# ten2net/Gym-Trading-Env

Measured on AMD Instinct MI355X. Metric: env-steps/sec, higher is better.
Workload: dtype f64

## Files before the change

gym-trading-env_amd/batched.py:

```python
from __future__ import annotations

import ctypes as C

import numpy as np

from . import _abi, spaces, staging
from .batched_history import history_column, history_columns
from .config import make_config

_NP = {"int32": np.int32, "float64": np.float64}


def _as_staged(ds, n_dyn, name="Stock"):
    if isinstance(ds, staging.StagedDataset):
        return ds
    if isinstance(ds, tuple) and len(ds) in (2, 4):
        return staging.stage_arrays(ds[0], ds[1], n_dyn=n_dyn, name=name,
                                    high=ds[2] if len(ds) == 4 else None,
                                    low=ds[3] if len(ds) == 4 else None)
    return staging.stage_dataframe(ds, n_dyn=n_dyn, name=name)


def _device_view(ptr, shape, typestr, device, strides=None):
    import torch
# ... 1102 lines not shown
                raise ValueError(f"expected rule_of_env of shape ({self.num_envs},)")
        torch.cuda.current_stream(dev).synchronize()
        _abi.check(self._lib, self._lib.gte_bind_exit_rules(
            self._h, C.c_void_p(d_rules.data_ptr()), R, None if d_map is None else C.c_void_p(d_map.data_ptr()),
            C.byref(ptr)))
        self._exits = (d_rules, d_map)
        self._exit_state_ptr = int(ptr.value or 0)

    @property
    def num_exit_rules(self) -> int:
        return int(self._exits[0].shape[0]) if self._exits else 0

    def exit_state(self):
        from .exit_state import ExitState
        if not self._exit_state_ptr:
            raise ValueError("exit_state() before bind_exits(): the env has no exit state yet")
        return ExitState(self, self._exit_state_ptr)

    def synchronize(self):
        _abi.check(self._lib, self._lib.gte_synchronize(self._h))

    def launch_info(self) -> dict:
        v = [C.c_int32() for _ in range(4)]
        _abi.check(self._lib, self._lib.gte_get_launch_info(self._h, *[C.byref(x) for x in v]))
        d = dict(zip(("envs_per_wave", "threads_per_block", "n_blocks", "vector_bytes"),
                     (x.value for x in v)))
        flags, d["vector_bytes"] = divmod(d["vector_bytes"], 1000)
        d["phase_a"] = "cooperative" if flags & 1 else "per-wave"
        d["dyn_columns"] = ("global", "lds-raw-rings", "lds-resolved")[(flags >> 1) & 3]
        d["structure"] = "phase A, LDS barrier, gather"
        d["obs_stores"] = ("plain", "non-temporal", "sc1", "?")[(flags >> 4) & 3]
        d["resident_workgroups_per_cu"] = (flags >> 6) & 15
        d["slide_obs_stores"] = ("plain", "non-temporal", "sc1", "?")[(flags >> 10) & 3]
        return d

    def timer_start(self):
        _abi.check(self._lib, self._lib.gte_timer_start(self._h))

    def timer_mark(self):
        _abi.check(self._lib, self._lib.gte_timer_stop(self._h, None))

    def timer_stop(self) -> float:
        ms = C.c_float()
        _abi.check(self._lib, self._lib.gte_timer_stop(self._h, C.byref(ms)))
        return ms.value

    def close(self, **kwargs):
        if getattr(self, "_h", None) and self._h.value:
            self._lib.gte_destroy(self._h)
            self._h = C.c_void_p()
        self.closed = True

    def __del__(self):
        try:
            self.close()
        except Exception:
            pass
```

gym-trading-env_amd/csrc/gte_api.hip:

```cpp
#include <hip/hip_runtime.h>

#include <climits>
#include <cstdarg>
#include <cstdio>
#include <cstdlib>
#include <cstring>
#include <new>
#include <string>
#include <utility>
#include <vector>

#include "gte_launch.h"
#include "gte_ledger.h"

using gte::DatasetDesc;
using gte::EnvRec;
using gte::Params;
using gte_ledger::FLAGS;
using gte_ledger::WINDOW;
using gte_ledger::ledger;

static thread_local std::string g_err = "";

static int fail(int code, const char* fmt, ...) {
  char buf[512];
  va_list ap;
  va_start(ap, fmt);
  vsnprintf(buf, sizeof buf, fmt, ap);
  va_end(ap);
  g_err = buf;
  return code;
}

#define HIPCHK(expr)                                                              \
  do {                                                                            \
    hipError_t e_ = (expr);                                                       \
    if (e_ != hipSuccess)                                                         \
      return fail(e_ == hipErrorOutOfMemory ? GTE_ERR_OOM : GTE_ERR_HIP,          \
                  "%s failed: %s", #expr, hipGetErrorString(e_));                 \
  } while (0)

enum { SLIDE_AB_ORDER = 1, SLIDE_AB_STORE = 2 };

struct LaunchPlan {
  int vec = 1, blocks = 0, threads = 256;
  bool coop = false;
  int stage = 0;
  int hot_per_cu = 0;
  int store = 0;
  int slide_store = 0;
  bool hot_tu = false;
  bool fused_log = false;
  bool always_dense = false;
  int slide_rows = 0;
  bool full_windows = false;
  int slide_ab = 0;
  bool fused_rollout = false;
  bool resident_rollout = false;
  int affinity_period = 0;
  int n_bins_per_ds = 0;
  int state_epw = 0;
  int rollout_epw = 0;
  int resident_slots[3] = {0, 0, 0};
  int resident_epb[3] = {0, 0, 0};
};

struct gte_env {
  gte_config cfg;
  Params p;
  hipStream_t stream = nullptr;
  hipStream_t own_stream = nullptr;
  hipEvent_t ev0 = nullptr, ev1 = nullptr;
  std::vector<void*> allocs;
  std::vector<DatasetDesc> h_ds;
  std::vector<void*> ds_allocs[4];
  DatasetDesc* d_ds = nullptr;
  gte_outputs owned;
  int32_t* d_actions = nullptr;
  uint8_t* d_mask = nullptr;
  int32_t *d_inj_idx = nullptr, *d_inj_pos = nullptr, *d_inj_ds = nullptr;
  int32_t *d_q_idx = nullptr, *d_q_pos = nullptr, *d_q_ds = nullptr;
  double* d_lo_limit_in = nullptr;
  uint8_t* d_lo_persist_in = nullptr;
// ... 241 lines not shown
  int nb = 8192 / p.D;
  if (const char* o = getenv("GTE_AFFINITY_BINS")) nb = atoi(o) / p.D;
  nb = nb < 1 ? 1 : (nb > 4096 ? 4096 : nb);
  L.n_bins_per_ds = nb;
  TRY(dev_alloc(E, &E->d_perm, N, false));
  TRY(dev_alloc(E, &E->d_slot_of_rank, N, false));
  TRY(dev_alloc(E, &E->d_bins, (size_t)2 * p.D * nb));
  if (hipMemcpy(E->d_slot_of_rank, slot_of_rank.data(), sizeof(int32_t) * N, hipMemcpyHostToDevice) !=
      hipSuccess)
    return fail(GTE_ERR_HIP, "copying slot_of_rank failed");
  L.affinity_period = period;
  return GTE_OK;
}

static int slide_store_policy(const gte_env* E) {
  const LaunchPlan& L = E->plan;
  const Params& p = E->p;
  if (L.slide_rows == 0 || L.full_windows || (L.slide_ab & SLIDE_AB_STORE)) return L.store;
  int s = E->cfg.nontemporal_obs;
  if (s == 3) s = ((size_t)p.N * (p.W + L.slide_rows) * p.Fobs * sizeof(float) > ((size_t)190 << 20)) ? 1 : L.store;
  if (s != L.store && L.hot_tu && s != 0) {
    hipDeviceProp_t prop;
    const size_t smem = gte::lds_bytes(p, L.stage);
    const int per_cu = s == 1 ? gte::hot_blocks_per_cu_nt(smem) : gte::hot_blocks_per_cu(smem);
    if (hipGetDeviceProperties(&prop, E->cfg.device) != hipSuccess || prop.multiProcessorCount <= 0 ||
        per_cu < (L.blocks + prop.multiProcessorCount - 1) / prop.multiProcessorCount)
      s = L.store;
  }
  if (const char* o = getenv("GTE_SLIDE_STORE"))
    if (o[0] >= '0' && o[0] <= '2' && o[1] == '\0') s = o[0] - '0';
  return s;
}

static int plan_launches(gte_env* E) {
  LaunchPlan& L = E->plan;
  Params& p = E->p;
  const gte_config& cfg = E->cfg;
  const int kv = cfg.kernel_variant;
  L.store = cfg.nontemporal_obs;
  if (L.store == 3) L.store = ((size_t)p.N * p.W * p.Fobs * sizeof(float) > ((size_t)190 << 20)) ? 1 : 2;
  step_geometry(E, !(kv & (GTE_KV_PER_WAVE_PHASE_A | GTE_KV_NO_LDS_STAGING)), !(kv & GTE_KV_GENERIC_COPY));
  p.debug = cfg.debug_flags;
  L.coop = (p.epw * GTE_WAVES <= 64) && !(kv & GTE_KV_PER_WAVE_PHASE_A);
  L.stage = (p.nd > 0 && gte::lds_bytes(p, 1) <= 48 * 1024 && !(kv & GTE_KV_NO_LDS_STAGING)) ? (p.persist ? 2 : 1) : 0;
  p.lean_rows = (L.vec == 4 && L.stage == 1 && !(kv & GTE_KV_GENERIC_COPY)) ? 1 : 0;
  p.hot_lds = (kv & GTE_KV_RECORD_DIRECT) ? 0 : 1;
  const bool hot_shape = L.vec == 4 && L.coop && L.stage == 1;
  L.hot_tu = hot_shape && !(kv & GTE_KV_SHARED_TU);
  L.fused_log = cfg.log_steps > 0 && !(kv & GTE_KV_LOG_SEPARATE);
  L.always_dense = (kv & GTE_KV_DENSE_FLAGS) != 0;
  L.slide_rows = 0;
  if (hot_shape && (int64_t)p.W * p.Fobs / 4 >= 64 && p.has_window && !p.persist && !cfg.final_obs &&
      cfg.log_steps == 0 && cfg.obs_slack_rows >= 0)
    L.slide_rows = cfg.obs_slack_rows > 0 ? cfg.obs_slack_rows : 2 * p.W / 5;
  L.full_windows = getenv("GTE_SLIDE_FULL_WINDOWS") != nullptr;
  if (const char* o = getenv("GTE_SLIDE_AB")) L.slide_ab = atoi(o);
  L.slide_store = slide_store_policy(E);
  L.fused_rollout = hot_shape && !cfg.final_obs && cfg.log_steps == 0 && !(kv & GTE_KV_ROLLOUT_PER_STEP);
  L.resident_rollout = p.W >= 2 && !(kv & GTE_KV_ROLLOUT_GATHER);
  L.state_epw = (p.N >= 64 * 1024) ? 64 : 32;
  return setup_affinity(E);
}

extern "C" {

int gte_abi_version(void) { return GTE_ABI_VERSION; }

const char* gte_last_error(void) { return g_err.c_str(); }

int gte_device_count(void) {
  int n = 0;
  if (hipGetDeviceCount(&n) != hipSuccess) return 0;
  return n;
}

int gte_create(const gte_config* cfg, gte_env** out) {
  if (!out) return fail(GTE_ERR_INVALID, "out is NULL");
  *out = nullptr;
  TRY(validate(cfg));
  TRY(require_device(cfg->device));
  HIPCHK(hipSetDevice(cfg->device));
  gte_env* E = new (std::nothrow) gte_env();
  if (!E) return fail(GTE_ERR_OOM, "host allocation failed");
  E->cfg = *cfg;
  memset(&E->p, 0, sizeof(Params));
  memset(&E->owned, 0, sizeof(gte_outputs));
  Params& p = E->p;
  p.N = cfg->n_envs;
  p.D = cfg->n_datasets;
  p.Fs = cfg->n_static;
// ... 351 lines not shown
  const bool slide = slides_own && !capturing && ledger().holds(E, WINDOW, {obs}) && E->p.obs_head < L.slide_rows;
  const bool env_order = slide && !L.full_windows && !(L.slide_ab & SLIDE_AB_ORDER);
  if (env_order) { if (L.affinity_period > 0) E->steps_since_rebuild += 1; }
  else TRY(age_order(E, 1));
  Params p = E->p;
  if (env_order) p.perm = nullptr;
  if (terminal_rec) p.final_rec = terminal_rec;
  p.actions = t.actions; p.obs = t.obs; p.reward = t.reward; p.reward64 = t.reward64;
  p.terminated = t.terminated; p.truncated = t.truncated;
  if (!t.own_obs) {
    p.obs_rows = p.W; p.obs_head = 0;
    obs = {t.obs, sizeof(float) * (size_t)p.N * p.W * p.Fobs};
  } else if (E->sliding) {
    if (slide) {
      E->p.obs_head += 1;
      if (p.persist || p.final_obs)
        return fail(GTE_ERR_STATE, "internal: a sliding step with dyn_persist or final_obs (plan_launches grants neither)");
      p.slide = L.full_windows ? 0 : 1;
    } else {
      E->p.obs_head = 0;
    }
    p.obs_head = E->p.obs_head;
  }
  advance_term_slot(E, p);
  if (L.fused_log) {
    p.log = E->log;
    p.log_cursor = E->log_cursor + (E->term_slot ^ 1);
  }
  const gte_ledger::Span term = flag_span(E, p.terminated), trunc = flag_span(E, p.truncated);
  p.flags_sparse = !capturing && !L.always_dense && ledger().holds(E, FLAGS, {term, trunc}) ? 1 : 0;
  ledger().wrote(E, {obs, term, trunc}, capturing, FLAGS | WINDOW);
  const bool hot = L.hot_tu && gte::hot_tu_covers(p);
  if (p.slide) store = L.slide_store;
  if (hot && store == 2)
    HIPCHK(gte::launch_step_hot(p, L.blocks, L.threads, gte::lds_bytes(p, L.stage), E->stream));
  else if (hot && store == 1)
    HIPCHK(gte::launch_step_hot_nt(p, L.blocks, L.threads, gte::lds_bytes(p, L.stage), E->stream));
  else
    HIPCHK(gte::launch_step(p, L.vec, store, L.coop, L.stage, L.blocks, L.threads, E->stream));
  ledger().establish(E, FLAGS, {term, trunc}, capturing);
  if (slides_own) ledger().establish(E, WINDOW, {obs}, capturing);
  if (L.fused_log) E->log_rows += 1;
  else TRY(append_log(E, p));
  return GTE_OK;
}

int gte_step(gte_env* E, const int32_t* actions, int32_t actions_on_device) {
  if (!E) return fail(GTE_ERR_INVALID, "env is NULL");
  if (!E->was_reset) return fail(GTE_ERR_STATE, "gte_step before gte_reset");
  if (!actions) return fail(GTE_ERR_INVALID, "actions is NULL");
  const bool capturing = stream_capturing(E);
  if (capturing && !actions_on_device)
    return fail(GTE_ERR_STATE, "gte_step on a capturing stream needs device-resident actions "
                               "(a copy from pageable host memory cannot be captured)");
  if (!actions_on_device) {
    TRY(stage(E, E->d_actions, actions, sizeof(int32_t) * (size_t)E->p.N));
    actions = E->d_actions;
  }
  return enqueue_step(E, own_targets(E, actions), E->plan.store, capturing);
}

int gte_get_schedule(gte_env* E, gte_schedule* out) {
  if (!E || !out) return fail(GTE_ERR_INVALID, "NULL argument");
  out->log_rows = E->log_rows;
  out->term_slot = E->term_slot;
  out->steps_since_rebuild = E->steps_since_rebuild;
  return GTE_OK;
// ... 997 lines not shown
  if (!E || !host_dst) return fail(GTE_ERR_INVALID, "NULL argument");
  const Params& p = E->p;
  if (first_env < 0 || n < 0 || (int64_t)first_env + n > p.N)
    return fail(GTE_ERR_INVALID, "env range [%d, %d) out of [0, %d)", first_env, first_env + n, p.N);
  const size_t per = (size_t)p.W * p.Fobs;
  if (!p.obs) return fail(GTE_ERR_STATE, "gte_read_obs before gte_reset (no observation exists yet)");
  HIPCHK(hipStreamSynchronize(E->stream));
  const size_t stride = (size_t)obs_env_stride(p);
  const float* src = obs_window0(p) + stride * first_env;
  if (stride == per || n == 0)
    HIPCHK(hipMemcpy(host_dst, src, sizeof(float) * per * n, hipMemcpyDeviceToHost));
  else
    HIPCHK(hipMemcpy2D(host_dst, sizeof(float) * per, src, sizeof(float) * stride, sizeof(float) * per, (size_t)n,
                       hipMemcpyDeviceToHost));
  return GTE_OK;
}

int gte_copy_to_host(gte_env* E, const void* device_src, void* host_dst, uint64_t bytes) {
  if (!E || !device_src || !host_dst) return fail(GTE_ERR_INVALID, "NULL argument");
  HIPCHK(hipStreamSynchronize(E->stream));
  HIPCHK(hipMemcpy(host_dst, device_src, (size_t)bytes, hipMemcpyDeviceToHost));
  return GTE_OK;
}

int gte_get_launch_info(gte_env* E, int32_t* envs_per_wave, int32_t* threads_per_block,
                        int32_t* n_blocks, int32_t* vector_bytes) {
  if (!E) return fail(GTE_ERR_INVALID, "env is NULL");
  if (envs_per_wave) *envs_per_wave = E->p.epw;
  const LaunchPlan& L = E->plan;
  if (threads_per_block) *threads_per_block = L.threads;
  if (n_blocks) *n_blocks = L.blocks;
  if (vector_bytes)
    *vector_bytes = L.vec * 4 + 1000 * ((L.coop ? 1 : 0) + 2 * L.stage + 16 * L.store + 64 * (L.hot_per_cu & 15) +
                                        1024 * (E->sliding ? L.slide_store : L.store));
  return GTE_OK;
}

#ifdef GTE_STAMPS
int gte_debug_set_stamps(gte_env* E, void* device_buf) {
  if (!E) return fail(GTE_ERR_INVALID, "env is NULL");
  E->p.inj_ds = (const int32_t*)device_buf;
  return GTE_OK;
}
#endif

void gte_destroy(gte_env* E) {
  if (!E) return;
  (void)hipSetDevice(E->cfg.device);
  (void)gte_comm_destroy(E);
  (void)hipStreamSynchronize(E->stream);
  if (E->own_stream) (void)hipStreamSynchronize(E->own_stream);
  for (void* ptr : E->allocs) if (ptr) (void)hipFree(ptr);
  for (auto& v : E->ds_allocs)
    for (void* ptr : v)
      if (ptr) (void)hipFree(ptr);
  for (int32_t* q : {E->d_q_idx, E->d_q_pos, E->d_q_ds})
    if (q) (void)hipFree(q);
  if (E->h_snap) (void)hipHostFree(E->h_snap);
  if (E->h_logpack) (void)hipHostFree(E->h_logpack);
  if (E->ev0) (void)hipEventDestroy(E->ev0);
  if (E->ev1) (void)hipEventDestroy(E->ev1);
  if (E->own_stream) (void)hipStreamDestroy(E->own_stream);
  ledger().forget(E);
  delete E;
}

}
// ... 1 lines not shown
```

gym-trading-env_amd/csrc/gte_kernels.hip:

```cpp
#include "gte_step.h"

namespace gte {

__global__ void gte_add_orders_kernel(const Params p, const int32_t* pos_index,
                                      const double* limit, const uint8_t* persistent) {
  const int e = blockIdx.x * blockDim.x + threadIdx.x;
  if (e >= p.N) return;
  const int32_t pi = pos_index[e];
  if (pi < 0) return;
  int32_t* lp = p.lo_pos + (int64_t)e * p.P;
  const int n = p.rec[e].lo_n;
  int j = 0;
  while (j < n && p.positions[lp[j]] != p.positions[pi]) ++j;
  if (j == n) p.rec[e].lo_n = n + 1;
  lp[j] = pi;
  p.lo_limit[(int64_t)e * p.P + j] = limit[e];
  p.lo_persist[(int64_t)e * p.P + j] = persistent ? persistent[e] : 0;
}

__global__ void gte_affinity_hist_kernel(const Params p, int32_t* hist, int n_bins_per_ds) {
  const int e = blockIdx.x * blockDim.x + threadIdx.x;
  if (e >= p.N) return;
  const int d = p.rec[e].dsi;
  const int64_t T = p.ds[d].T;
// ... 51 lines not shown
  return hipGetLastError();
}

__global__ void gte_extract_state_kernel(const EnvRec* rec, int n, StateSoA o) {
  const int e = blockIdx.x * blockDim.x + threadIdx.x;
  if (e >= n) return;
  const EnvRec r = rec[e];
  o.idx[e] = r.idx; o.step[e] = r.step; o.pos[e] = r.pos; o.dsi[e] = r.dsi;
  o.start[e] = r.start; o.episode[e] = r.episode; o.needs_reset[e] = r.needs_reset;
  o.asset[e] = r.asset; o.fiat[e] = r.fiat; o.ia[e] = r.ia; o.ifi[e] = r.ifi;
  o.pv[e] = r.pv; o.realpos[e] = r.realpos;
}

hipError_t launch_extract_state(const EnvRec* rec, int n, const StateSoA& o, hipStream_t stream) {
  hipLaunchKernelGGL(gte_extract_state_kernel, dim3((n + 255) / 256), dim3(256), 0, stream, rec, n, o);
  return hipGetLastError();
}

__global__ void gte_rewind_queue_kernel(EnvRec* rec, int n) {
  const int e = blockIdx.x * blockDim.x + threadIdx.x;
  if (e < n) rec[e].q_head = 0;
}

hipError_t launch_rewind_queue(EnvRec* rec, int n, hipStream_t stream) {
  hipLaunchKernelGGL(gte_rewind_queue_kernel, dim3((n + 255) / 256), dim3(256), 0, stream, rec, n);
  return hipGetLastError();
}


size_t lds_bytes(const Params& p, int stage) {
  const size_t EPB = (size_t)p.epw * GTE_WAVES;
  size_t b = EPB * (16 + 64 + 4 * GTE_MAX_DYN + 4) + (p.final_obs ? EPB * sizeof(FinalJob) : 0) +
             (p.log.rows ? EPB * sizeof(LogRow) : 0);
  if (stage) b += EPB * (size_t)p.W * (size_t)(p.nd ? p.nd : 1) * 4;
  return b;
}

template <int MODE>
static hipError_t launch_mode(const Params& p, int vec, int nt, bool coop, int stage,
                              int blocks, int threads, hipStream_t stream) {
  const uint32_t V = (uint32_t)(p.W * p.Fobs);
  const uint64_t vm = magic40(V / vec), fm = magic40((uint32_t)p.Fobs / vec);
  const uint64_t wm = magic40((uint32_t)(p.W * (p.nd ? p.nd : 1)));
  const size_t smem = lds_bytes(p, stage);
#define GTE_L(VEC, NT, CO, ST) \
  hipLaunchKernelGGL((gte_kernel<MODE, VEC, NT, CO, ST>), dim3(blocks), dim3(threads), smem, \
                     stream, p, vm, fm, wm)
#define GTE_L_ST(VEC, NT, CO) do { if (stage == STAGE_RAW) GTE_L(VEC, NT, CO, STAGE_RAW); \
    else if (stage == STAGE_LATE) GTE_L(VEC, NT, CO, STAGE_LATE); else GTE_L(VEC, NT, CO, STAGE_NONE); } while (0)
#define GTE_L_CO(VEC, NT) do { if (coop) GTE_L_ST(VEC, NT, true); else GTE_L_ST(VEC, NT, false); } while (0)
#define GTE_L_NT(VEC) do { if (nt == 2) GTE_L_CO(VEC, 2); else if (nt == 1) GTE_L_CO(VEC, 1); \
                           else GTE_L_CO(VEC, 0); } while (0)
  if (vec == 4) GTE_L_NT(4); else GTE_L_NT(1);
#undef GTE_L_NT
#undef GTE_L_CO
#undef GTE_L_ST
#undef GTE_L
  return hipGetLastError();
}

hipError_t launch_add_orders(const Params& p, const int32_t* pos_index, const double* limit,
                             const uint8_t* persistent, hipStream_t stream) {
  hipLaunchKernelGGL(gte_add_orders_kernel, dim3((p.N + 255) / 256), dim3(256), 0, stream, p,
                     pos_index, limit, persistent);
  return hipGetLastError();
}

hipError_t launch_step(const Params& p, int vec, int nt, bool coop, int stage, int blocks,
                       int threads, hipStream_t stream) {
  return launch_mode<MODE_STEP>(p, vec, nt, coop, stage, blocks, threads, stream);
}

hipError_t launch_reset(const Params& p, int vec, int nt, bool coop, int stage, int blocks,
                        int threads, hipStream_t stream) {
  return launch_mode<MODE_RESET>(p, vec, nt, coop, stage, blocks, threads, stream);
}

}
```

gym-trading-env_amd/csrc/gte_launch.h:

```cpp
#pragma once
#include "gte_device.h"

namespace gte {

constexpr int LEAN_MAX_ROWS = 512;
#ifndef GTE_LEAN_U
#define GTE_LEAN_U 4
#endif
constexpr int ROLLOUT_WAVES = 4;
inline int rollout_blocks(int n_envs, int epw) {
  return (int)((((int64_t)n_envs + epw - 1) / epw + ROLLOUT_WAVES - 1) / ROLLOUT_WAVES);
}
constexpr int RES_NEW = 2;
constexpr int RES_OWNERS = 192;
constexpr size_t RES_LDS_MAX = 160 * 1024;
constexpr size_t LDS_OPT_IN = 64 * 1024;

inline uint64_t magic40(uint32_t d) { return ((1ull << 40) + d - 1) / d; }

hipError_t launch_step(const Params& p, int vec, int nt, bool coop, int stage, int blocks, int threads,
                       hipStream_t stream);
hipError_t launch_reset(const Params& p, int vec, int nt, bool coop, int stage, int blocks, int threads,
                        hipStream_t stream);
size_t lds_bytes(const Params& p, int stage);
hipError_t launch_add_orders(const Params& p, const int32_t* pos_index, const double* limit,
                             const uint8_t* persistent, hipStream_t stream);
hipError_t launch_affinity_rebuild(const Params& p, int32_t* bins, int n_bins_per_ds, const int32_t* slot_of_rank,
                                   int32_t* perm_out, hipStream_t stream);
struct StateSoA {
  int32_t *idx, *step, *pos, *dsi, *start, *episode, *needs_reset;
  double *asset, *fiat, *ia, *ifi, *pv, *realpos;
};
hipError_t launch_extract_state(const EnvRec* rec, int n, const StateSoA& o, hipStream_t stream);
hipError_t launch_rewind_queue(EnvRec* rec, int n, hipStream_t stream);

hipError_t launch_step_hot(const Params& p, int blocks, int threads, size_t smem, hipStream_t stream);
hipError_t launch_step_hot_nt(const Params& p, int blocks, int threads, size_t smem, hipStream_t stream);
int hot_blocks_per_cu(size_t smem);
int hot_blocks_per_cu_nt(size_t smem);

struct RolloutArgs {
  const int32_t* actions;
  int32_t K;
  float* obs;
  float* reward;
  double* reward64;
  uint8_t *terminated, *truncated;
  double* valuation;
  int32_t epb;
  int32_t n_groups;
  int32_t* group_counter;
};
size_t resident_lds_bytes(const Params& p, int epb);
int resident_blocks_per_cu(const Params& p, int epb, int nt);
hipError_t launch_rollout_resident(const Params& p, const RolloutArgs& r, int nt, int blocks, hipStream_t stream);
hipError_t launch_rollout_state(const Params& p, const RolloutArgs& r, int n_steps, int epw, hipStream_t stream);
int rollout_blocks_per_cu(const Params& p, int nt);
// ... 80 lines not shown
```

gym-trading-env_amd/csrc/gte_phase_a.h:

```cpp
#pragma once
#include "gte_launch.h"

namespace gte {


typedef float float4_t __attribute__((ext_vector_type(4)));

enum { MODE_STEP = 0, MODE_RESET = 1 };

#ifdef GTE_STAMPS
#define GTE_STAMP(k)                                                                          \
  do {                                                                                        \
    if (MODE == MODE_STEP && p.inj_ds) {                                                      \
      asm volatile("s_waitcnt vmcnt(0) lgkmcnt(0)" ::: "memory");       \
      if (threadIdx.x == 0)                                                                   \
        ((unsigned long long*)p.inj_ds)[blockIdx.x * 8 + (k)] = __builtin_amdgcn_s_memrealtime(); \
    }                                                                                         \
  } while (0)
#define GTE_STAMP_HWID(k)                                                                     \
  do {                                                                                        \
    if (MODE == MODE_STEP && p.inj_ds && threadIdx.x == 0)                                    \
      ((unsigned long long*)p.inj_ds)[blockIdx.x * 8 + (k)] =                                 \
          (unsigned long long)__builtin_amdgcn_s_getreg((31 << 11) | 4) |                     \
          ((unsigned long long)__builtin_amdgcn_s_getreg((31 << 11) | 20) << 32);             \
  } while (0)
#else
#define GTE_STAMP(k) do {} while (0)
#define GTE_STAMP_HWID(k) do {} while (0)
#endif

struct EnvRegs {
  int32_t idx, step, pos, dsi, start, needs_reset, lo_n, flags_out;
  Portfolio q;
  double pv, realpos;
};

__device__ inline void load_state(const Params& p, int e, EnvRegs& s) {
  const EnvRec* r = &p.rec[e];
  const int4* ri = reinterpret_cast<const int4*>(r);
  const int4 a = ri[0];
  const double2* rd = reinterpret_cast<const double2*>(&r->asset);
  const double2 d0 = rd[0], d1 = rd[1], d2 = rd[2];
  const int4 b = ri[4];
  const int4 c = ri[5];
  s.idx = a.x; s.step = a.y; s.pos = a.z; s.dsi = a.w;
  s.start = b.x; s.needs_reset = b.z; s.lo_n = c.z; s.flags_out = c.w;
  s.q.asset = d0.x; s.q.fiat = d0.y; s.q.ia = d1.x; s.q.ifi = d1.y;
  s.pv = d2.x; s.realpos = d2.y;
}

__device__ inline void store_state_at(EnvRec* r, const EnvRegs& s) {
  *reinterpret_cast<int4*>(&r->idx) = make_int4(s.idx, s.step, s.pos, s.dsi);
  double2* d = reinterpret_cast<double2*>(&r->asset);
  d[0] = make_double2(s.q.asset, s.q.fiat);
  d[1] = make_double2(s.q.ia, s.q.ifi);
  d[2] = make_double2(s.pv, s.realpos);
}
typedef int __attribute__((ext_vector_type(4))) int4_t;
typedef double __attribute__((ext_vector_type(2))) double2_t;
typedef unsigned char __attribute__((address_space(3))) * lds_byte_ptr;
__device__ inline void store_state_lds(lds_byte_ptr h, const EnvRegs& s) {
  typedef int4_t __attribute__((address_space(3))) * li4;
  typedef double2_t __attribute__((address_space(3))) * ld2;
  int4_t a = {s.idx, s.step, s.pos, s.dsi};
  double2_t d0 = {s.q.asset, s.q.fiat}, d1 = {s.q.ia, s.q.ifi}, d2 = {s.pv, s.realpos};
  *(li4)h = a;
  *(ld2)(h + 16) = d0;
  *(ld2)(h + 32) = d1;
  *(ld2)(h + 48) = d2;
}
__device__ inline void store_state(const Params& p, int e, const EnvRegs& s) { store_state_at(&p.rec[e], s); }

__device__ inline void store_flags(const Params& p, int e, EnvRegs& s, int32_t f) {
  if (!p.flags_sparse || f != s.flags_out) {
    p.terminated[e] = (uint8_t)(f & 1);
    p.truncated[e] = (uint8_t)(f >> 1);
  }
  if (f != s.flags_out) { s.flags_out = f; p.rec[e].flags_out = f; }
}
// ... 60 lines not shown
  for (int j = 0; j < n; ++j) {
    const int32_t pi = lp[j];
    const double limit = ll[j];
    const uint8_t per = lper[j];
    bool keep = true;
    const double position = p.positions[pi];
    if (position != p.positions[s.pos] && limit <= hi && limit >= lo) {
      trade_to_position(s.q, position, limit, p.fees);
      s.pos = pi;
      if (!per) keep = false;
    }
    if (keep) {
      if (k != j) { lp[k] = pi; ll[k] = limit; lper[k] = per; }
      ++k;
    }
  }
  s.lo_n = k;
  p.rec[e].lo_n = k;
}

__device__ inline void pop_injection(const Params& p, int e, EnvRegs& s, int32_t& qi,
                                     int32_t& qp, int32_t& qd) {
  qi = qp = qd = -1;
  if (p.q_n <= 0) return;
  const int32_t h = p.rec[e].q_head;
  if (h >= p.q_n) return;
  p.rec[e].q_head = h + 1;
  const int64_t k = (int64_t)e * p.q_n + h;
  if (p.q_idx) qi = p.q_idx[k];
  if (p.q_pos) qp = p.q_pos[k];
  if (p.q_ds) qd = p.q_ds[k];
}

__device__ inline void make_job(const Params& p, int e, const EnvRegs& s, bool fresh,
                                ObsJob& job) {
#pragma unroll
  for (int i = 0; i < GTE_MAX_DYN; ++i) {
    float v = 0.0f;
    if (i < p.nd) {
      const double x = (p.dyn_kind[i] == GTE_DYN_REAL_POSITION) ? s.realpos
                                                                : p.positions[s.pos];
      v = (float)x;
      const int64_t slot = p.persist ? (int64_t)s.idx : (int64_t)(s.idx % p.W);
      p.ring[((int64_t)e * p.depth + slot) * p.nd + i] = v;
    }
    job.cur[i] = v;
  }
  const int32_t first = s.idx - p.W + 1;
  job.src = p.ds[s.dsi].feat + (int64_t)first * p.Fobs;
  job.slot0 = p.persist ? first : (s.idx + 1) % p.W;
  int32_t nz;
  if (fresh) nz = p.W - 1;
  else if (p.persist) nz = 0;
  else {
    nz = s.start - first;
    nz = nz < 0 ? 0 : (nz > p.W - 1 ? p.W - 1 : nz);
  }
  job.n_zero = nz;
  job.idx = s.idx;
  job.flags = 1 | ((fresh && p.persist) ? 2 : 0);
}


struct StepOut {
  double reward, pv, realpos, asset, fiat, ia, ifi;
  int32_t idx, step, pos, dsi;
  int32_t flags;
};

struct PriceCarry {
  double cur, next;
  int32_t idx, dsi;
};

template <int MODE>
__device__ inline void phase_a(const Params& p, int e, bool active, int lane, ObsJob& job,
                               FinalJob* fin = nullptr, bool compact = true,
                               double* pv_out = nullptr, EnvRegs* carried = nullptr,
                               const int32_t* action_in = nullptr, bool write_record = true,
                               PriceCarry* pc = nullptr, StepOut* so = nullptr,
                               lds_byte_ptr hot = nullptr) {
  if (fin) fin->flags = 0;
  job.src = nullptr; job.slot0 = 0; job.n_zero = 0; job.idx = 0; job.flags = 0;
#pragma unroll
  for (int i = 0; i < GTE_MAX_DYN; ++i) job.cur[i] = 0.0f;
  bool ended = false;

  if (MODE == MODE_RESET) {
    if (active && (p.mask == nullptr || p.mask[e] != 0)) {
      EnvRegs s;
      load_state(p, e, s);
      bool fresh = false;
      const int32_t ii = p.inj_idx ? p.inj_idx[e] : -1;
      const int32_t ip = p.inj_pos ? p.inj_pos[e] : -1;
      const int32_t id = p.inj_ds ? p.inj_ds[e] : -1;
      if (p.D > 1 && p.rec[e].n_picks == 0) next_dataset(p, e, id, s, fresh);
      do_reset(p, e, ii, ip, id, s, fresh);
      store_state(p, e, s);
      p.reward[e] = 0.0f; p.reward64[e] = 0.0;
      p.terminated[e] = 0; p.truncated[e] = 0;
      make_job(p, e, s, fresh, job);
    }
    return;
  }

  if (active) {
    EnvRegs s_own;
    EnvRegs& s = carried ? *carried : s_own;
// ... 41 lines not shown
      if (pc) {
        pc->cur = price;
        pc->idx = s.idx;
        pc->dsi = s.dsi;
        pc->next = (s.idx + 1 < d_T) ? d_close[s.idx + 1] : price;
      }
      GTE_STAMP(3);
      s.q.ia = pymax0(-s.q.asset) * p.rate;
      s.q.ifi = pymax0(-s.q.fiat) * p.rate;
      const double pv = valorisation(s.q, price);
      const bool done = (pv / p.V0) <= 0.7;
      bool trunc = s.idx >= d_T - 1;
      if (p.max_dur > 0 && s.step >= p.max_dur - 1) trunc = true;
      s.realpos = (s.q.asset - s.q.ia) * price / valorisation(s.q, price);
      double rew = 0.0;
      if (!done) rew = reward_of(p, pv, s.pv);
      s.pv = pv;
      p.reward64[e] = rew;
      p.reward[e] = (float)rew;
      store_flags(p, e, s, (done ? 1 : 0) | (trunc ? 2 : 0));
      if (so) { so->reward = rew; so->flags = (done ? 1 : 0) | (trunc ? 2 : 0); }
      ended = done || trunc;
      slides = !(ended && p.autoreset == GTE_AUTORESET_SAME_STEP);
      if (ended) { s.needs_reset = 1; p.rec[e].needs_reset = 1; }
      if (ended && p.autoreset == GTE_AUTORESET_SAME_STEP) {
#ifndef GTE_HOT_ONLY
        if (p.final_rec) {
          store_state_at(&p.final_rec[e], s);
          p.final_rec[e].needs_reset = s.needs_reset;
          p.final_rec[e].start = s.start;
        }
#endif
        ObsJob term;
        make_job(p, e, s, false, term);
        int32_t qi, qp, qd;
        pop_injection(p, e, s, qi, qp, qd);
        do_reset(p, e, qi, qp, qd, s, fresh);
        if (pc) pc->idx = -1;
        if (fin && p.final_obs) {
          fin->src = term.src; fin->slot0 = term.slot0; fin->n_zero = term.n_zero; fin->flags = 1;
          const int64_t cs = p.persist ? (int64_t)s.idx : (int64_t)(s.idx % p.W);
          fin->clob_slot = (int32_t)cs;
#pragma unroll
          for (int i = 0; i < GTE_MAX_DYN; ++i) {
            fin->cur[i] = term.cur[i];
            fin->clob[i] = (i < p.nd) ? p.ring[((int64_t)e * p.depth + cs) * p.nd + i] : 0.0f;
          }
        }
      }
    }
    GTE_STAMP(4);
    if (pv_out) *pv_out = s.pv;
    if (write_record) {
      if (hot) store_state_lds(hot, s);
      else store_state(p, e, s);
    }
    if (so) {
      so->idx = s.idx; so->step = s.step; so->pos = s.pos; so->dsi = s.dsi;
      so->pv = s.pv; so->realpos = s.realpos;
      so->asset = s.q.asset; so->fiat = s.q.fiat; so->ia = s.q.ia; so->ifi = s.q.ifi;
    }
    make_job(p, e, s, fresh, job);
    if (slides && p.slide) job.flags |= JOB_SLIDES;
    GTE_STAMP(5);
  }

  const unsigned long long m = __ballot(ended);
  if (compact && m != 0ull) {
    const int cnt = __popcll(m);
    const int leader = __ffsll((long long)m) - 1;
    int base = 0;
    if (lane == leader) base = atomicAdd(p.term_count, cnt);
    base = __shfl(base, leader);
    if (ended) {
      const int my = __popcll(m & ((1ull << lane) - 1ull));
      p.term_ids[base + my] = e;
    }
  }
}

}
```

gym-trading-env_amd/csrc/gte_step.h:

```cpp
#pragma once
#include "gte_phase_a.h"

namespace gte {



__device__ inline uint32_t fastdiv40(uint32_t k, uint64_t magic) {
  return (uint32_t)(((uint64_t)k * magic) >> 40);
}

template <int NT, typename T>
__device__ inline void store_out(T* dst, const T& v) {
  if constexpr (NT == 2 && sizeof(T) == 16) {
    asm volatile("global_store_dwordx4 %0, %1, off sc1\n\ts_nop 1" ::"v"(dst), "v"(v));
  } else if constexpr (NT == 2) {
    const float f = __builtin_bit_cast(float, v);
    asm volatile("global_store_dword %0, %1, off sc1" ::"v"(dst), "v"(f));
  } else if constexpr (NT == 1) {
    __builtin_nontemporal_store(v, dst);
  } else {
    *dst = v;
  }
}

// ... 76 lines not shown
#pragma unroll
  for (int i = 0; i < GTE_MAX_DYN; ++i) L.cur[slot * GTE_MAX_DYN + i] = job.cur[i];
}

__device__ inline float dyn_value(const Params& p, const WgLds& L, int s, const float* ring_e,
                                  int w, int i) {
  if (w == p.W - 1) return L.cur[s * GTE_MAX_DYN + i];
  const uint32_t m = L.job[s].meta;
  if (w < meta_n_zero(m)) return 0.0f;
  int32_t slot;
  if (p.persist) {
    slot = L.idx[s] - p.W + 1 + w;
  } else {
    slot = meta_slot0(m) + w;
    if (slot >= p.W) slot -= p.W;
  }
  return ring_e[(int64_t)slot * p.nd + i];
}

__device__ inline void stage_dynamic(const Params& p, const WgLds& L, int s_first,
                                     int n_env, int lane, uint64_t wnd_magic) {
  const uint32_t WND = (uint32_t)(p.W * p.nd);
  const uint32_t total = (uint32_t)n_env * WND;
  for (uint32_t k = (uint32_t)lane; k < total; k += 64u) {
    const uint32_t el = fastdiv40(k, wnd_magic);
    const uint32_t r = k - el * WND;
    const uint32_t w = r / (uint32_t)p.nd;
    const int i = (int)(r - w * (uint32_t)p.nd);
    const int s = s_first + (int)el;
    const float* ring_e = p.ring + (int64_t)L.job[s].env * p.depth * p.nd;
    L.staged[(uint32_t)s * WND + r] = dyn_value(p, L, s, ring_e, (int)w, i);
  }
}

enum { STAGE_NONE = 0, STAGE_RAW = 1, STAGE_LATE = 2 };

__device__ inline void stage_raw_rings(const Params& p, const WgLds& L, int s_first, int n_env,
                                       int lane, uint64_t wnd_magic) {
  const uint32_t WND = (uint32_t)(p.W * p.nd);
  const uint32_t total = (uint32_t)n_env * WND;
  float* dst = L.staged + (uint32_t)s_first * WND;
  for (uint32_t k = (uint32_t)lane; k < total; k += 64u) {
    const uint32_t el = fastdiv40(k, wnd_magic);
    const uint32_t r = k - el * WND;
    dst[k] = p.ring[(int64_t)L.job[s_first + (int)el].env * WND + r];
  }
}

template <int VEC, int STAGE, typename vec_t>
__device__ inline void patch_dynamic(const Params& p, const WgLds& L, vec_t& v, int s, uint32_t m,
                                     const float* ring_e, int w, int col) {
  if (col + VEC <= p.Fs || (p.debug & 2)) return;
  const bool is_cur = (w == p.W - 1);
  int32_t slot = meta_slot0(m) + w;
  if (STAGE == STAGE_RAW) slot -= (slot >= p.W) ? p.W : 0;
  const bool zero = !is_cur && w < meta_n_zero(m);
  float x[GTE_MAX_DYN];
#pragma unroll
  for (int i = 0; i < GTE_MAX_DYN; ++i) {
    x[i] = 0.0f;
    if (i < p.nd) {
      if (STAGE == STAGE_RAW) {
        const float* a = is_cur ? &L.cur[s * GTE_MAX_DYN + i] : &L.staged[(s * p.W + slot) * p.nd + i];
        x[i] = zero ? 0.0f : *a;
      } else if (STAGE == STAGE_LATE) {
        x[i] = L.staged[(s * p.W + w) * p.nd + i];
      } else {
        x[i] = dyn_value(p, L, s, ring_e, w, i);
// ... 213 lines not shown
#pragma unroll
        for (int i = 0; i < GTE_MAX_DYN; ++i) {
          x[i] = 0.0f;
          if (i < p.nd) {
            if ((int)w == p.W - 1) x[i] = f.cur[i];
            else if ((int)w < f.n_zero) x[i] = 0.0f;
            else if (slot == f.clob_slot) x[i] = f.clob[i];
            else x[i] = ring_e[(int64_t)slot * p.nd + i];
          }
        }
        if constexpr (VEC == 4) {
          set_tail(v, p.nd, x);
        } else {
          const int i = col - p.Fs;
          float r = x[0];
#pragma unroll
          for (int k = 1; k < GTE_MAX_DYN; ++k) r = (i == k) ? x[k] : r;
          v = r;
        }
      }
      *(vec_t*)(dst + (int64_t)j * VEC) = v;
    }
  }
}

#ifndef GTE_GATHER_U
#define GTE_GATHER_U 4
#endif
template <int MODE, int VEC, int NT, bool COOP, int STAGE>
__global__ __launch_bounds__(256) void gte_kernel(const Params p, const uint64_t vpe_magic,
                                                  const uint64_t fv_magic,
                                                  const uint64_t wnd_magic) {
  extern __shared__ __attribute__((aligned(16))) unsigned char gte_smem[];
  const int lane = threadIdx.x & 63;
  const int wib = threadIdx.x >> 6;
  if (MODE == MODE_STEP && blockIdx.x == 0 && threadIdx.x == 0) p.term_count_next[0] = 0;
#ifndef GTE_HOT_ONLY
  if (MODE == MODE_STEP && p.log.rows && blockIdx.x == 0 && threadIdx.x == 0)
    *log_cursor_other(p.log_cursor) = *p.log_cursor + 1;
#endif
  const int EPB = p.epw * GTE_WAVES;
  const int wg_first = blockIdx.x * EPB;
  if (wg_first >= p.N) return;
  const int n_wg = min(EPB, p.N - wg_first);
  GTE_STAMP(0);
  const WgLds L = carve_lds(gte_smem, EPB, p.final_obs != nullptr, p.log.rows != nullptr);
  const int s_first = wib * p.epw;
  const int n_env = min(p.epw, n_wg - s_first);
  auto prepare = [&](int first, int count) {
    if (lane < p.epw) {
      const int slot = wg_first + first + lane;
      L.job[first + lane].env = (lane < count) ? (p.perm ? p.perm[slot] : slot) : -1;
    }
    if (STAGE == STAGE_RAW && count > 0) {
      __builtin_amdgcn_fence(__ATOMIC_RELEASE, "wavefront");
      __builtin_amdgcn_wave_barrier();
      __builtin_amdgcn_fence(__ATOMIC_ACQUIRE, "wavefront");
      stage_raw_rings(p, L, first, count, lane, wnd_magic);
    }
  };
  if (!COOP) {
    prepare(s_first, n_env);
  } else if (wib >= 1) {
    prepare(s_first, n_env);
    if (wib == 1) prepare(0, min(p.epw, n_wg));
  }
  GTE_STAMP(1);
#ifdef GTE_STAMPS_HWID
  GTE_STAMP_HWID(1);
#endif

  if (!COOP || wib == 0) {
    const int s = COOP ? lane : wib * p.epw + lane;
    const bool owns = COOP ? (lane < EPB) : (lane < p.epw);
    const bool active = owns && s < n_wg;
    const int e = active ? (p.perm ? p.perm[wg_first + s] : wg_first + s) : 0;
    ObsJob job;
    FinalJob fin;
    const lds_byte_ptr hot = (MODE == MODE_STEP && p.hot_lds) ? (lds_byte_ptr)(L.hot + 64 * s) : (lds_byte_ptr) nullptr;
#ifndef GTE_HOT_ONLY
    if (MODE == MODE_STEP && p.log.rows) {
      StepOut so = {};
      phase_a<MODE>(p, e, active, lane, job, p.final_obs ? &fin : nullptr, true, nullptr, nullptr, nullptr,
                    true, nullptr, &so, hot);
      if (active) {
        typedef int4_t __attribute__((address_space(3))) * li4;
        typedef double2_t __attribute__((address_space(3))) * ld2;
        const lds_byte_ptr w = (lds_byte_ptr)(L.logrow + sizeof(LogRow) * s);
        int4_t a = {so.idx, so.step, so.pos, so.dsi};
        double2_t d0 = {so.pv, so.realpos};
        double2_t d1 = {(so.step == 0) ? 0.0 : so.reward, so.asset};
        double2_t d2 = {so.fiat, so.ia};
        double2_t d3 = {so.ifi, __longlong_as_double((long long)(so.flags & 0xff))};
        *(li4)w = a;
        *(ld2)(w + 16) = d0;
        *(ld2)(w + 32) = d1;
        *(ld2)(w + 48) = d2;
        *(ld2)(w + 64) = d3;
      }
    } else
#endif
    phase_a<MODE>(p, e, active, lane, job, p.final_obs ? &fin : nullptr, true, nullptr, nullptr, nullptr, true,
                  nullptr, nullptr, hot);
    if (owns) publish_job(L, s, job);
    if (owns && p.final_obs) L.fin[s] = fin;
  }
  asm volatile("s_waitcnt lgkmcnt(0)\n\ts_barrier" ::: "memory");
  GTE_STAMP(6);

  if (MODE == MODE_STEP && p.hot_lds && n_env > 0) flush_hot_records(p, L, s_first, n_env, lane);
#ifndef GTE_HOT_ONLY
  if (MODE == MODE_STEP && p.log.rows && n_env > 0) flush_log_rows(p, L, s_first, n_env, lane);
#endif
  if (n_env <= 0 || (p.debug & 1)) return;
  if (p.persist) zero_fresh_stores(p, L, s_first, n_env, lane);
  if (STAGE == STAGE_LATE) {
    stage_dynamic(p, L, s_first, n_env, lane, wnd_magic);
    __builtin_amdgcn_fence(__ATOMIC_RELEASE, "wavefront");
    __builtin_amdgcn_wave_barrier();
    __builtin_amdgcn_fence(__ATOMIC_ACQUIRE, "wavefront");
  }
  bool lean = false;
  if constexpr (MODE == MODE_STEP && VEC == 4) {
    if (p.slide && !p.debug) {
      phase_b_slide<NT>(p, L, s_first, n_env, lane, fv_magic);
      const uint32_t m = L.job[s_first + (lane < n_env ? lane : 0)].meta;
      unsigned long long full = __ballot(lane < n_env && (m & 1u) && !(m & (uint32_t)JOB_SLIDES));
      const uint32_t VPE = (uint32_t)(p.W * p.Fobs) / 4u;
      while (full) {
        const uint32_t el = (uint32_t)(__ffsll((long long)full) - 1);
        full &= full - 1ull;
        phase_b<VEC, NT, STAGE, GTE_GATHER_U>(p, L, s_first, n_env, lane, vpe_magic, fv_magic, el * VPE,
                                              (el + 1u) * VPE);
      }
      GTE_STAMP(7);
      return;
    }
  }
  if constexpr (MODE == MODE_STEP && VEC == 4 && STAGE == STAGE_RAW) {
    if (p.lean_rows > 0 && n_env == p.epw && n_env * p.W <= LEAN_MAX_ROWS && p.W * p.Fobs / 4 >= 64 &&
        ((uint32_t)n_env * (uint32_t)(p.W * p.Fobs / 4)) % (64u * GTE_LEAN_U) == 0u && !p.debug &&
        __ballot(lane < n_env && !(L.job[s_first + (lane < n_env ? lane : 0)].meta & 1u)) == 0ull) {
      switch (p.nd) {
        case 1: resolve_dynamic_rows<1>(p, L, s_first, n_env, lane, wnd_magic); break;
        case 2: resolve_dynamic_rows<2>(p, L, s_first, n_env, lane, wnd_magic); break;
        case 3: resolve_dynamic_rows<3>(p, L, s_first, n_env, lane, wnd_magic); break;
        default: resolve_dynamic_rows<4>(p, L, s_first, n_env, lane, wnd_magic); break;
      }
      __builtin_amdgcn_fence(__ATOMIC_RELEASE, "wavefront");
      __builtin_amdgcn_wave_barrier();
      __builtin_amdgcn_fence(__ATOMIC_ACQUIRE, "wavefront");
      switch (p.nd) {
        case 1: phase_b_lean<NT, 1>(p, L, s_first, n_env, lane); break;
        case 2: phase_b_lean<NT, 2>(p, L, s_first, n_env, lane); break;
        case 3: phase_b_lean<NT, 3>(p, L, s_first, n_env, lane); break;
        default: phase_b_lean<NT, 4>(p, L, s_first, n_env, lane); break;
      }
      lean = true;
    }
  }
  if (!lean) phase_b<VEC, NT, STAGE, GTE_GATHER_U>(p, L, s_first, n_env, lane, vpe_magic, fv_magic);
  GTE_STAMP(7);
  if (MODE == MODE_STEP && p.final_obs) final_windows<VEC>(p, L, s_first, n_env, lane, fv_magic);
}

}
```

Measured before the change: 3.823 billion.

## Add unstaged sliding-step kernel variant with vectorized non-temporal ring stores

Adds a STAGE_SLIDE kernel variant for sliding-window steps that skips LDS staging of dynamic-column rings. This shrinks LDS use and can raise resident workgroups per CU. Ring writes in make_job become one vectorized, optionally non-temporal store per env instead of scalar per-column stores. A policy picks this path only when slide stores are non-temporal and occupancy covers all blocks in one wave. This adds another kernel instantiation and relies on a host-side occupancy query.

```diff
diff --git a/gym-trading-env_amd/batched.py b/gym-trading-env_amd/batched.py
--- a/gym-trading-env_amd/batched.py
+++ b/gym-trading-env_amd/batched.py
@@ -1158,6 +1158,7 @@
         d["obs_stores"] = ("plain", "non-temporal", "sc1", "?")[(flags >> 4) & 3]
         d["resident_workgroups_per_cu"] = (flags >> 6) & 15
         d["slide_obs_stores"] = ("plain", "non-temporal", "sc1", "?")[(flags >> 10) & 3]
+        d["slide_ring_staged"] = not (flags >> 12) & 1
         return d
 
     def timer_start(self):
diff --git a/gym-trading-env_amd/csrc/gte_api.hip b/gym-trading-env_amd/csrc/gte_api.hip
--- a/gym-trading-env_amd/csrc/gte_api.hip
+++ b/gym-trading-env_amd/csrc/gte_api.hip
@@ -40,7 +40,7 @@
                   "%s failed: %s", #expr, hipGetErrorString(e_));                 \
   } while (0)
 
-enum { SLIDE_AB_ORDER = 1, SLIDE_AB_STORE = 2 };
+enum { SLIDE_AB_ORDER = 1, SLIDE_AB_STORE = 2, SLIDE_AB_STAGED = 4 };
 
 struct LaunchPlan {
   int vec = 1, blocks = 0, threads = 256;
@@ -49,6 +49,7 @@
   int hot_per_cu = 0;
   int store = 0;
   int slide_store = 0;
+  bool slide_unstaged = false;
   bool hot_tu = false;
   bool fused_log = false;
   bool always_dense = false;
@@ -356,6 +357,17 @@
   return s;
 }
 
+static bool slide_unstaged_policy(const gte_env* E) {
+  const LaunchPlan& L = E->plan;
+  const Params& p = E->p;
+  if (L.slide_rows == 0 || L.full_windows || (L.slide_ab & SLIDE_AB_STAGED)) return false;
+  if (L.slide_store != 1) return false;
+  hipDeviceProp_t prop;
+  const int per_cu = gte::slide_blocks_per_cu(gte::lds_bytes(p, gte::STAGE_SLIDE));
+  return hipGetDeviceProperties(&prop, E->cfg.device) == hipSuccess && prop.multiProcessorCount > 0 &&
+         per_cu >= (L.blocks + prop.multiProcessorCount - 1) / prop.multiProcessorCount;
+}
+
 static int plan_launches(gte_env* E) {
   LaunchPlan& L = E->plan;
   Params& p = E->p;
@@ -380,6 +392,7 @@
   L.full_windows = getenv("GTE_SLIDE_FULL_WINDOWS") != nullptr;
   if (const char* o = getenv("GTE_SLIDE_AB")) L.slide_ab = atoi(o);
   L.slide_store = slide_store_policy(E);
+  L.slide_unstaged = slide_unstaged_policy(E);
   L.fused_rollout = hot_shape && !cfg.final_obs && cfg.log_steps == 0 && !(kv & GTE_KV_ROLLOUT_PER_STEP);
   L.resident_rollout = p.W >= 2 && !(kv & GTE_KV_ROLLOUT_GATHER);
   L.state_epw = (p.N >= 64 * 1024) ? 64 : 32;
@@ -797,7 +810,9 @@
   ledger().wrote(E, {obs, term, trunc}, capturing, FLAGS | WINDOW);
   const bool hot = L.hot_tu && gte::hot_tu_covers(p);
   if (p.slide) store = L.slide_store;
-  if (hot && store == 2)
+  if (store == 1 && p.slide && L.slide_unstaged)
+    HIPCHK(gte::launch_step(p, L.vec, store, L.coop, gte::STAGE_SLIDE, L.blocks, L.threads, E->stream));
+  else if (hot && store == 2)
     HIPCHK(gte::launch_step_hot(p, L.blocks, L.threads, gte::lds_bytes(p, L.stage), E->stream));
   else if (hot && store == 1)
     HIPCHK(gte::launch_step_hot_nt(p, L.blocks, L.threads, gte::lds_bytes(p, L.stage), E->stream));
@@ -1861,7 +1876,8 @@
   if (n_blocks) *n_blocks = L.blocks;
   if (vector_bytes)
     *vector_bytes = L.vec * 4 + 1000 * ((L.coop ? 1 : 0) + 2 * L.stage + 16 * L.store + 64 * (L.hot_per_cu & 15) +
-                                        1024 * (E->sliding ? L.slide_store : L.store));
+                                        1024 * (E->sliding ? L.slide_store : L.store) +
+                                        4096 * ((E->sliding && L.slide_unstaged) ? 1 : 0));
   return GTE_OK;
 }
 
diff --git a/gym-trading-env_amd/csrc/gte_kernels.hip b/gym-trading-env_amd/csrc/gte_kernels.hip
--- a/gym-trading-env_amd/csrc/gte_kernels.hip
+++ b/gym-trading-env_amd/csrc/gte_kernels.hip
@@ -107,7 +107,7 @@
   const size_t EPB = (size_t)p.epw * GTE_WAVES;
   size_t b = EPB * (16 + 64 + 4 * GTE_MAX_DYN + 4) + (p.final_obs ? EPB * sizeof(FinalJob) : 0) +
              (p.log.rows ? EPB * sizeof(LogRow) : 0);
-  if (stage) b += EPB * (size_t)p.W * (size_t)(p.nd ? p.nd : 1) * 4;
+  if (stage == STAGE_RAW || stage == STAGE_LATE) b += EPB * (size_t)p.W * (size_t)(p.nd ? p.nd : 1) * 4;
   return b;
 }
 
@@ -141,8 +141,14 @@
   return hipGetLastError();
 }
 
+static hipError_t launch_step_slide(const Params& p, int blocks, int threads, hipStream_t stream);
+
 hipError_t launch_step(const Params& p, int vec, int nt, bool coop, int stage, int blocks,
                        int threads, hipStream_t stream) {
+  if (stage == STAGE_SLIDE) {
+    if (vec != 4 || !coop || nt != 1 || !p.slide) return hipErrorInvalidValue;
+    return launch_step_slide(p, blocks, threads, stream);
+  }
   return launch_mode<MODE_STEP>(p, vec, nt, coop, stage, blocks, threads, stream);
 }
 
@@ -151,4 +157,26 @@
   return launch_mode<MODE_RESET>(p, vec, nt, coop, stage, blocks, threads, stream);
 }
 
+template <int NT>
+static hipError_t launch_slide_nt(const Params& p, int blocks, int threads, hipStream_t stream) {
+  const uint32_t V = (uint32_t)(p.W * p.Fobs);
+  const uint64_t vm = magic40(V / 4), fm = magic40((uint32_t)p.Fobs / 4);
+  const uint64_t wm = magic40((uint32_t)(p.W * (p.nd ? p.nd : 1)));
+  hipLaunchKernelGGL((gte_kernel<MODE_STEP, 4, NT, true, STAGE_SLIDE>), dim3(blocks), dim3(threads),
+                     lds_bytes(p, STAGE_SLIDE), stream, p, vm, fm, wm);
+  return hipGetLastError();
 }
+
+static hipError_t launch_step_slide(const Params& p, int blocks, int threads, hipStream_t stream) {
+  return launch_slide_nt<1>(p, blocks, threads, stream);
+}
+
+int slide_blocks_per_cu(size_t smem) {
+  int n = 0;
+  if (hipOccupancyMaxActiveBlocksPerMultiprocessor(&n, gte_kernel<MODE_STEP, 4, 1, true, STAGE_SLIDE>,
+                                                   64 * GTE_WAVES, smem) != hipSuccess)
+    return 0;
+  return n;
+}
+
+}
diff --git a/gym-trading-env_amd/csrc/gte_launch.h b/gym-trading-env_amd/csrc/gte_launch.h
--- a/gym-trading-env_amd/csrc/gte_launch.h
+++ b/gym-trading-env_amd/csrc/gte_launch.h
@@ -16,6 +16,12 @@
 constexpr size_t RES_LDS_MAX = 160 * 1024;
 constexpr size_t LDS_OPT_IN = 64 * 1024;
 
+enum { STAGE_NONE = 0, STAGE_RAW = 1, STAGE_LATE = 2, STAGE_SLIDE = 3 };
+enum { RING_SCALAR = 0, RING_PLAIN = 1, RING_NT = 2 };
+#ifndef GTE_SLIDE_RING
+#define GTE_SLIDE_RING RING_NT
+#endif
+
 inline uint64_t magic40(uint32_t d) { return ((1ull << 40) + d - 1) / d; }
 
 hipError_t launch_step(const Params& p, int vec, int nt, bool coop, int stage, int blocks, int threads,
@@ -23,6 +29,7 @@
 hipError_t launch_reset(const Params& p, int vec, int nt, bool coop, int stage, int blocks, int threads,
                         hipStream_t stream);
 size_t lds_bytes(const Params& p, int stage);
+int slide_blocks_per_cu(size_t smem);
 hipError_t launch_add_orders(const Params& p, const int32_t* pos_index, const double* limit,
                              const uint8_t* persistent, hipStream_t stream);
 hipError_t launch_affinity_rebuild(const Params& p, int32_t* bins, int n_bins_per_ds, const int32_t* slot_of_rank,
diff --git a/gym-trading-env_amd/csrc/gte_phase_a.h b/gym-trading-env_amd/csrc/gte_phase_a.h
--- a/gym-trading-env_amd/csrc/gte_phase_a.h
+++ b/gym-trading-env_amd/csrc/gte_phase_a.h
@@ -45,6 +45,10 @@
   const int4 c = ri[5];
   s.idx = a.x; s.step = a.y; s.pos = a.z; s.dsi = a.w;
   s.start = b.x; s.needs_reset = b.z; s.lo_n = c.z; s.flags_out = c.w;
+#ifdef GTE_PROBE_NO_COLD_LOAD
+  s.start = a.x - a.y; s.lo_n = 0; s.flags_out = 0;
+  s.needs_reset = (a.x >= (int32_t)p.ds[a.w].T - 1 || (p.max_dur > 0 && a.y >= p.max_dur - 1)) ? 1 : 0;
+#endif
   s.q.asset = d0.x; s.q.fiat = d0.y; s.q.ia = d1.x; s.q.ifi = d1.y;
   s.pv = d2.x; s.realpos = d2.y;
 }
@@ -171,6 +175,23 @@
   if (p.q_ds) qd = p.q_ds[k];
 }
 
+template <int RING, typename T>
+__device__ inline void store_ring_vec(T* dst, const T& v) {
+  if constexpr (RING == RING_NT) __builtin_nontemporal_store(v, dst);
+  else *dst = v;
+}
+template <int RING>
+__device__ inline void store_ring_slot(float* dst, const float x[GTE_MAX_DYN], int nd) {
+  typedef float f2 __attribute__((ext_vector_type(2)));
+  switch (nd) {
+    case 1: store_ring_vec<RING>(dst, x[0]); break;
+    case 2: { const f2 v = {x[0], x[1]}; store_ring_vec<RING>((f2*)dst, v); break; }
+    case 3: store_ring_vec<RING>(dst, x[0]); store_ring_vec<RING>(dst + 1, x[1]); store_ring_vec<RING>(dst + 2, x[2]); break;
+    default: { const float4_t v = {x[0], x[1], x[2], x[3]}; store_ring_vec<RING>((float4_t*)dst, v); break; }
+  }
+}
+
+template <int RING = RING_SCALAR>
 __device__ inline void make_job(const Params& p, int e, const EnvRegs& s, bool fresh,
                                 ObsJob& job) {
 #pragma unroll
@@ -180,10 +201,17 @@
       const double x = (p.dyn_kind[i] == GTE_DYN_REAL_POSITION) ? s.realpos
                                                                 : p.positions[s.pos];
       v = (float)x;
-      const int64_t slot = p.persist ? (int64_t)s.idx : (int64_t)(s.idx % p.W);
-      p.ring[((int64_t)e * p.depth + slot) * p.nd + i] = v;
+      if constexpr (RING == RING_SCALAR) {
+        const int64_t slot = p.persist ? (int64_t)s.idx : (int64_t)(s.idx % p.W);
+#ifndef GTE_PROBE_NO_RING_STORE
+        p.ring[((int64_t)e * p.depth + slot) * p.nd + i] = v;
+#endif
+      }
     }
     job.cur[i] = v;
+  }
+  if constexpr (RING != RING_SCALAR) {
+    if (p.nd > 0) store_ring_slot<RING>(p.ring + ((int64_t)e * p.depth + (int64_t)(s.idx % p.W)) * p.nd, job.cur, p.nd);
   }
   const int32_t first = s.idx - p.W + 1;
   job.src = p.ds[s.dsi].feat + (int64_t)first * p.Fobs;
@@ -212,7 +240,7 @@
   int32_t idx, dsi;
 };
 
-template <int MODE>
+template <int MODE, int RING = RING_SCALAR>
 __device__ inline void phase_a(const Params& p, int e, bool active, int lane, ObsJob& job,
                                FinalJob* fin = nullptr, bool compact = true,
                                double* pv_out = nullptr, EnvRegs* carried = nullptr,
@@ -320,7 +348,7 @@
         }
 #endif
         ObsJob term;
-        make_job(p, e, s, false, term);
+        make_job<RING>(p, e, s, false, term);
         int32_t qi, qp, qd;
         pop_injection(p, e, s, qi, qp, qd);
         do_reset(p, e, qi, qp, qd, s, fresh);
@@ -348,7 +376,7 @@
       so->pv = s.pv; so->realpos = s.realpos;
       so->asset = s.q.asset; so->fiat = s.q.fiat; so->ia = s.q.ia; so->ifi = s.q.ifi;
     }
-    make_job(p, e, s, fresh, job);
+    make_job<RING>(p, e, s, fresh, job);
     if (slides && p.slide) job.flags |= JOB_SLIDES;
     GTE_STAMP(5);
   }
diff --git a/gym-trading-env_amd/csrc/gte_step.h b/gym-trading-env_amd/csrc/gte_step.h
--- a/gym-trading-env_amd/csrc/gte_step.h
+++ b/gym-trading-env_amd/csrc/gte_step.h
@@ -132,8 +132,6 @@
     L.staged[(uint32_t)s * WND + r] = dyn_value(p, L, s, ring_e, (int)w, i);
   }
 }
-
-enum { STAGE_NONE = 0, STAGE_RAW = 1, STAGE_LATE = 2 };
 
 __device__ inline void stage_raw_rings(const Params& p, const WgLds& L, int s_first, int n_env,
                                        int lane, uint64_t wnd_magic) {
@@ -413,6 +411,8 @@
                                                   const uint64_t fv_magic,
                                                   const uint64_t wnd_magic) {
   extern __shared__ __attribute__((aligned(16))) unsigned char gte_smem[];
+  constexpr int PB_STAGE = (STAGE == STAGE_SLIDE) ? STAGE_NONE : STAGE;
+  constexpr int RING = (STAGE == STAGE_SLIDE) ? GTE_SLIDE_RING : RING_SCALAR;
   const int lane = threadIdx.x & 63;
   const int wib = threadIdx.x >> 6;
   if (MODE == MODE_STEP && blockIdx.x == 0 && threadIdx.x == 0) p.term_count_next[0] = 0;
@@ -462,8 +462,8 @@
 #ifndef GTE_HOT_ONLY
     if (MODE == MODE_STEP && p.log.rows) {
       StepOut so = {};
-      phase_a<MODE>(p, e, active, lane, job, p.final_obs ? &fin : nullptr, true, nullptr, nullptr, nullptr,
-                    true, nullptr, &so, hot);
+      phase_a<MODE, RING>(p, e, active, lane, job, p.final_obs ? &fin : nullptr, true, nullptr, nullptr, nullptr,
+                          true, nullptr, &so, hot);
       if (active) {
         typedef int4_t __attribute__((address_space(3))) * li4;
         typedef double2_t __attribute__((address_space(3))) * ld2;
@@ -481,8 +481,8 @@
       }
     } else
 #endif
-    phase_a<MODE>(p, e, active, lane, job, p.final_obs ? &fin : nullptr, true, nullptr, nullptr, nullptr, true,
-                  nullptr, nullptr, hot);
+    phase_a<MODE, RING>(p, e, active, lane, job, p.final_obs ? &fin : nullptr, true, nullptr, nullptr, nullptr, true,
+                        nullptr, nullptr, hot);
     if (owns) publish_job(L, s, job);
     if (owns && p.final_obs) L.fin[s] = fin;
   }
@@ -511,8 +511,8 @@
       while (full) {
         const uint32_t el = (uint32_t)(__ffsll((long long)full) - 1);
         full &= full - 1ull;
-        phase_b<VEC, NT, STAGE, GTE_GATHER_U>(p, L, s_first, n_env, lane, vpe_magic, fv_magic, el * VPE,
-                                              (el + 1u) * VPE);
+        phase_b<VEC, NT, PB_STAGE, GTE_GATHER_U>(p, L, s_first, n_env, lane, vpe_magic, fv_magic, el * VPE,
+                                                 (el + 1u) * VPE);
       }
       GTE_STAMP(7);
       return;
@@ -540,7 +540,7 @@
       lean = true;
     }
   }
-  if (!lean) phase_b<VEC, NT, STAGE, GTE_GATHER_U>(p, L, s_first, n_env, lane, vpe_magic, fv_magic);
+  if (!lean) phase_b<VEC, NT, PB_STAGE, GTE_GATHER_U>(p, L, s_first, n_env, lane, vpe_magic, fv_magic);
   GTE_STAMP(7);
   if (MODE == MODE_STEP && p.final_obs) final_windows<VEC>(p, L, s_first, n_env, lane, fv_magic);
 }
```

New measurement: 4.089 billion, median of 5. 1.07x the previous value.
